# MrGiovanni/R-Super

Hardware: AMD Instinct MI355X
Metric: CT voxels/sec/node (96³ patch, bs=2/GPU) (higher is better)
Workload: dtype bf16; 1 GPU; R-Super 3D UNet(base 32, 26 classes, BasicBlock/IN) full training step (fwd + masked BCE + Dice loss + bwd + clip + AdamW + EMA), 96^3 patches, batch 2/GPU (BASELINE.json configs[1]); global_batch=2, patch=96, parallelism=dp1, sanity_checks_form=device-side flags read one step late (train_ddp.StepGuard)

## Files before the change

include/rsuper_hip.h:

```cpp
#ifndef RSUPER_HIP_H
#define RSUPER_HIP_H
#include <stddef.h>
#include <stdint.h>
#ifdef __cplusplus
extern "C" {
#endif

#define RSUPER_F32 0
#define RSUPER_BF16 1
#define RSUPER_OK 0
#define RSUPER_ERR_ARG 1
#define RSUPER_ERR_LAUNCH 2
#define RSUPER_ERR_UNSUPPORTED 3
#define RSUPER_ERR_NO_DEVICE 4

const char* rsuper_version(void);
int rsuper_device_check(void);


size_t rsuper_conv3_packed_elems(int dtype, int ka, int kb, int n_cols, int bn);

int rsuper_conv3_pack_weights(int dtype, int mode, const float* wa, const float* wb, int ka, int kb, int na, int nb,
                              int bn, void* packed, void* stream);

// ... 76 lines not shown
int rsuper_maxpool2_fwd(int dtype, const void* x, int ldx, void* y, int ldy, float* part, int blocks,
                        int N, int D, int H, int W, int C, void* stream);
int rsuper_maxpool2_bwd(int dtype, const void* x, int ldx, const void* dy, int lddy, void* dx, int lddx,
                        int N, int D, int H, int W, int C, void* stream);
int rsuper_maxpool2_bwd_add(int dtype, const void* x, int ldx, const void* dy, int lddy, const void* add, int lda, void* dx, int lddx,
                            int N, int D, int H, int W, int C, void* stream);

int rsuper_subsample2_fwd(int dtype, const void* x, int ldx, void* y, int ldy, float* part, int blocks,
                          int N, int D, int H, int W, int C, void* stream);
int rsuper_subsample2_bwd(int dtype, const void* dy, int lddy, void* dx, int lddx, int N, int D, int H, int W, int C, void* stream);

int rsuper_upsample_fwd(int dtype, const void* x, int ldx, void* y, int ldy, float* part, int blocks,
                        int N, int ID, int IH, int IW, int OD, int OH, int OW, int C, void* stream);
int rsuper_upsample_bwd(int dtype, const void* dy, int lddy, void* dx, int lddx,
                        int N, int ID, int IH, int IW, int OD, int OH, int OW, int C, void* stream);

int rsuper_stem_fwd(int dtype, const float* x, const float* w, void* y, int ldy, float* part,
                    int N, int D, int H, int W, int C, void* stream);
int rsuper_stem_wgrad(int dtype, const float* x, const void* dy, int lddy, float* dw, int N, int D, int H, int W, int C, void* stream);

int rsuper_head_fwd(int dtype, const void* x, int ldx, const float* w, const float* b, float* logits, int N, int vox, int C, int K, void* stream);
int rsuper_head_bwd_data(int dtype, const float* dlogits, const float* w, void* dx, int lddx, int N, int vox, int C, int K, void* stream);
int rsuper_head_bwd_weight(int dtype, const void* x, int ldx, const float* dlogits, float* dw, float* db, int N, int vox, int C, int K, void* stream);
int rsuper_head_bwd(int dtype, const void* x, int ldx, const float* dlogits, const float* w, void* dx, int lddx, float* dw, float* db,
                    int N, int vox, int C, int K, void* stream);

int rsuper_plane_partials_fwd(const float* x, size_t xstride, const uint8_t* t, const uint8_t* k, const float* w1, const uint8_t* w2,
                              double* sums, int flags, int planes, size_t V, void* stream);
int rsuper_plane_partials_bwd(const float* x, size_t xstride, const uint8_t* t, const uint8_t* k, const float* w1, const uint8_t* w2,
                              const float* g, float* dx, int flags, int planes, size_t V, void* stream);
// ... 174 lines not shown
```

r-super_amd/csrc/api.hip:

```cpp
#include <string.h>
#include <math.h>
#include <stdlib.h>
#include "common.hpp"
#include "kernels.hpp"
#include "misc.hpp"
#include "loss.hpp"
#include "morph.hpp"
#include "optim.hpp"
#include "../../include/rsuper_hip.h"

#define ST(s) ((hipStream_t)(s))

static inline bool dt_ok(int dt) { return dt == RS_F32 || dt == RS_BF16; }
static inline bool ch_ok(int C, int ld) { return C >= 0 && (C % 8) == 0 && (ld % 8) == 0 && ld >= C; }
static inline bool bn_ok(int bn) { return bn == 32 || bn == 64 || bn == 96 || bn == 128; }
static inline int ntiles_for(int n_cols, int bn) { const int per = bn / 32; return ((n_cols + bn - 1) / bn) * per; }
static inline int pack_cols(int mode, int na, int nb) { return mode == 1 ? (nb ? (nb & 0xFFFF) : na) : na + nb; }
static inline bool pack_range_ok(int mode, int na, int nb) { return mode != 1 || nb == 0 || ((nb >> 16) % 32 == 0 && (nb & 0xFFFF) > 0 && (nb >> 16) + (nb & 0xFFFF) <= na); }

#include "igemm_plan.hpp"

template <typename F>
static int for_chunks(int n, void* const* p, void* const* g, void* const* m, void* const* v, void* const* e, const size_t* numel, F f) {
    for (int i0 = 0; i0 < n; i0 += RS_MT_MAX) {
// ... 400 lines not shown
    return rs_launch_subsample(p, dtype, 1, 1, ST(stream));
}

int rsuper_upsample_fwd(int dtype, const void* x, int ldx, void* y, int ldy, float* part, int blocks,
                        int N, int ID, int IH, int IW, int OD, int OH, int OW, int C, void* stream) {
    if (!dt_ok(dtype) || !x || !y || !ch_ok(C, ldx) || !ch_ok(C, ldy) || blocks <= 0) return RS_ERR_ARG;
    UpParams p = {x, ldx, y, ldy, nullptr, 0, part, N, ID, IH, IW, OD, OH, OW, C};
    return rs_launch_upsample(p, dtype, 0, blocks, ST(stream));
}
int rsuper_upsample_bwd(int dtype, const void* dy, int lddy, void* dx, int lddx,
                        int N, int ID, int IH, int IW, int OD, int OH, int OW, int C, void* stream) {
    if (!dt_ok(dtype) || !dy || !dx || !ch_ok(C, lddy) || !ch_ok(C, lddx)) return RS_ERR_ARG;
    UpParams p = {nullptr, 0, (void*)dy, lddy, dx, lddx, nullptr, N, ID, IH, IW, OD, OH, OW, C};
    return rs_launch_upsample(p, dtype, 1, 1, ST(stream));
}
int rsuper_stem_fwd(int dtype, const float* x, const float* w, void* y, int ldy, float* part,
                    int N, int D, int H, int W, int C, void* stream) {
    if (!dt_ok(dtype) || !x || !w || !y || !part || !ch_ok(C, ldy)) return RS_ERR_ARG;
    StemParams p = {x, w, y, ldy, part, nullptr, N, D, H, W, C};
    return rs_launch_stem(p, dtype, 0, ST(stream));
}
int rsuper_stem_wgrad(int dtype, const float* x, const void* dy, int lddy, float* dw, int N, int D, int H, int W, int C, void* stream) {
    if (!dt_ok(dtype) || !x || !dy || !dw || !ch_ok(C, lddy)) return RS_ERR_ARG;
    StemParams p = {x, nullptr, (void*)dy, lddy, nullptr, dw, N, D, H, W, C};
    return rs_launch_stem(p, dtype, 1, ST(stream));
}

int rsuper_head_fwd(int dtype, const void* x, int ldx, const float* w, const float* b, float* logits, int N, int vox, int C, int K, void* stream) {
    if (!dt_ok(dtype) || !x || !w || !b || !logits || !ch_ok(C, ldx) || K <= 0) return RS_ERR_ARG;
    HeadParams p = {x, ldx, w, b, logits, nullptr, 0, nullptr, nullptr, N, vox, C, K};
// ... 342 lines not shown
```

r-super_amd/csrc/misc.hpp:

```cpp
#pragma once
#include <hip/hip_runtime.h>
#include <stddef.h>
#include <stdint.h>

struct InBwdParams {
    const void* g; int ldg;
    const void* x; int ldx;
    const float* mr;
    const float* gm;
    const void* add1; int lda1;
    const void* add2; int lda2;
    void* out; int ldo;
    int N, vox, C;
};

struct PoolParams {
    const void* x; int ldx;
    void* y; int ldy;
    void* dx; int lddx;
    float* part;
    int N, D, H, W, C;
    const void* add; int lda;
};

struct UpParams {
    const void* x; int ldx;
    void* y; int ldy;
    void* dx; int lddx;
    float* part;
    int N, ID, IH, IW, OD, OH, OW, C;
};

struct StemParams {
    const float* x;
    const float* w;
    void* y; int ldy;
    float* part;
    float* dw;
    int N, D, H, W, C;
};

struct HeadParams {
    const void* x; int ldx;
    const float* w; const float* b;
    float* logits;
// ... 15 lines not shown
                         float* hbuf, float* y, int N, long vox, int C, int r, hipStream_t st);
int rs_launch_se_backward(const float* x, const float* dy, const float* ident, const float* w1, const float* w2, const float* ms, const float* tab,
                          const float* hbuf, float* part, float* gm, float* dz1buf, float* tab2, float* dx, float* dw1, float* db1, float* dw2,
                          float* db2, int N, long vox, int C, int r, hipStream_t st);
int rs_launch_cl_planar(const float* src, float* dst, int N, long vox, int C, int K, int dir, hipStream_t st);
int rs_depthwise_rows(long vox);
int rs_launch_depthwise(const float* x, const float* w, float* y, int N, int D, int H, int W, int C, int flip, hipStream_t st);
int rs_launch_depthwise_wgrad(const float* x, const float* dy, float* part, float* dw, int N, int D, int H, int W, int C, hipStream_t st);
int rs_launch_stats_finalize(const float* part, int N, int nblk, int C, double cnt, float eps, int mode, int split, float* out, hipStream_t st);
int rs_elem_blocks(size_t items);
int rs_glue_variant(int v);
int rs_launch_in_bwd(const InBwdParams& p, int dtype, hipStream_t st);
int rs_launch_pool(const PoolParams& p, int dtype, int bwd, int blocks, hipStream_t st);
int rs_launch_subsample(const PoolParams& p, int dtype, int bwd, int blocks, hipStream_t st);
int rs_launch_upsample(const UpParams& p, int dtype, int bwd, int blocks, hipStream_t st);
int rs_launch_stem(const StemParams& p, int dtype, int wgrad, hipStream_t st);
int rs_launch_head(const HeadParams& p, int dtype, int which, hipStream_t st);
```

r-super_amd/csrc/unet_misc.hip:

```cpp
#include <string.h>
#include "common.hpp"
#include "kernels.hpp"
#include "misc.hpp"

namespace {

__global__ __launch_bounds__(1024) void stats_finalize_kernel(const float* part, int nblk, int C, double cnt, float eps, int mode, int split, float* out) {
    __shared__ double red[32][32][2];
    const int n = blockIdx.y;
    const int cl = threadIdx.x & 31, g = threadIdx.x >> 5;
    const int c = blockIdx.x * 32 + cl;
    double s0 = 0.0, s1 = 0.0;
    if (c < C) {
        const float* base = part + ((size_t)n * nblk * C + c) * 2;
        int b = g;
        for (; b + 96 < nblk; b += 128) {
            const float2 v0 = *(const float2*)(base + (size_t)b * C * 2), v1 = *(const float2*)(base + (size_t)(b + 32) * C * 2);
            const float2 v2 = *(const float2*)(base + (size_t)(b + 64) * C * 2), v3 = *(const float2*)(base + (size_t)(b + 96) * C * 2);
            s0 += ((double)v0.x + (double)v1.x) + ((double)v2.x + (double)v3.x);
            s1 += ((double)v0.y + (double)v1.y) + ((double)v2.y + (double)v3.y);
        }
        for (; b < nblk; b += 32) {
            const float2 v = *(const float2*)(base + (size_t)b * C * 2);
            s0 += (double)v.x; s1 += (double)v.y;
// ... 420 lines not shown
    return w;
}

struct UpAxis { int lo, n; float w[6]; };
__device__ __forceinline__ UpAxis up_axis(int i, float scale, int I, int O) {
    UpAxis a;
    int hi;
    up_range(i, scale, O, a.lo, hi);
    a.n = hi - a.lo + 1;
    if (a.n > 6) a.n = 6;
#pragma unroll
    for (int k = 0; k < 6; ++k) a.w[k] = k < a.n ? up_weight(a.lo + k, i, scale, I) : 0.f;
    return a;
}

template <typename T>
__global__ void upsample_bwd_kernel(UpParams p) {
    constexpr int KP = Elem<T>::KP;
    const int CV = p.C / KP;
    const int n = blockIdx.y;
    const size_t total = (size_t)p.ID * p.IH * p.IW * CV;
    const int ovox = p.OD * p.OH * p.OW;
    const float sd = p.OD > 1 ? (float)(p.ID - 1) / (float)(p.OD - 1) : 0.f;
    const float sh = p.OH > 1 ? (float)(p.IH - 1) / (float)(p.OH - 1) : 0.f;
    const float sw = p.OW > 1 ? (float)(p.IW - 1) / (float)(p.OW - 1) : 0.f;
    for (size_t i = (size_t)blockIdx.x * blockDim.x + threadIdx.x; i < total; i += (size_t)gridDim.x * blockDim.x) {
        const int s = (int)(i % CV); const int v = (int)(i / CV);
        const int iw = v % p.IW, ih = (v / p.IW) % p.IH, id = v / (p.IW * p.IH);
        const UpAxis ad = up_axis(id, sd, p.ID, p.OD), ah = up_axis(ih, sh, p.IH, p.OH), aw = up_axis(iw, sw, p.IW, p.OW);
        float acc[KP];
// ... 6 lines not shown
            for (int b = 0; b < 6; ++b) {
                if (ah.w[b] == 0.f) continue;
                const float wdh = ad.w[a] * ah.w[b];
                const size_t rowo = (size_t)n * ovox + ((size_t)(ad.lo + a) * p.OH + (ah.lo + b)) * p.OW;
#pragma unroll
                for (int c = 0; c < 6; ++c) {
                    if (aw.w[c] == 0.f) continue;
                    float g[KP];
                    unpack16<T>(*(const uint4*)((const T*)p.y + (rowo + aw.lo + c) * p.ldy + s * KP), g);
                    const float wt = wdh * aw.w[c];
#pragma unroll
                    for (int j = 0; j < KP; ++j) acc[j] += wt * g[j];
                }
            }
        }
        *(uint4*)((T*)p.dx + ((size_t)n * p.ID * p.IH * p.IW + v) * p.lddx + s * KP) = pack16<T>(acc);
    }
}

template <typename T>
__global__ __launch_bounds__(256) void upsample_fwd2_kernel(UpParams p) {
    constexpr int KP = Elem<T>::KP;
    const int CV = p.C / KP, VL = 256 / CV;
    const int vl = threadIdx.x / CV, s = threadIdx.x % CV;
    const bool active = vl < VL;
    const int n = blockIdx.y;
    const int ovox = p.OD * p.OH * p.OW;
    const int per_blk = (ovox + gridDim.x - 1) / gridDim.x;
    const int v0 = blockIdx.x * per_blk, v1 = min(ovox, v0 + per_blk);
    const float sd = p.OD > 1 ? (float)(p.ID - 1) / (float)(p.OD - 1) : 0.f;
// ... 187 lines not shown
                for (int c = 0; c < NW; ++c) {
                    const uint32_t off = c < nc ? ((rowo + c) * (uint32_t)p.ldy + s * KP) * (uint32_t)sizeof(T) : 0xFFFFFFFFu;
                    const auto r = __builtin_amdgcn_raw_buffer_load_b128(rs, off, 0, 0);
                    q[c] = make_uint4(r[0], r[1], r[2], r[3]);
                }
#pragma unroll
                for (int c = 0; c < NW; ++c) {
                    float g[KP];
                    unpack16<T>(q[c], g);
                    const float wt = wdh * wc[c];
#pragma unroll
                    for (int j = 0; j < KP; ++j) acc[j] = fmaf(wt, g[j], acc[j]);
                }
            }
        }
        *(uint4*)((T*)p.dx + ((size_t)n * p.ID * p.IH * p.IW + v) * p.lddx + s * KP) = pack16<T>(acc);
    }
}

template <typename T>
__global__ __launch_bounds__(256) void upsample_bwd2_kernel(UpParams p) {
    extern __shared__ __attribute__((aligned(16))) char smem[];
    UpEnt* tab = (UpEnt*)smem;
    __shared__ int nwmax;
    if (threadIdx.x == 0) nwmax = 0;
    __syncthreads();
    const float sd = p.OD > 1 ? (float)(p.ID - 1) / (float)(p.OD - 1) : 0.f;
    const float sh = p.OH > 1 ? (float)(p.IH - 1) / (float)(p.OH - 1) : 0.f;
    const float sw = p.OW > 1 ? (float)(p.IW - 1) / (float)(p.OW - 1) : 0.f;
    for (int t = threadIdx.x; t < p.ID + p.IH + p.IW; t += 256) {
// ... 26 lines not shown
    }
    __syncthreads();
    const UpEnt* td = tab; const UpEnt* th = tab + p.ID; const UpEnt* tw = tab + p.ID + p.IH;
    const uint32_t CV = (uint32_t)p.C / Elem<T>::KP;
    const uint32_t total = (uint32_t)(p.ID * p.IH * p.IW) * CV;
    const uint32_t i0 = blockIdx.x * 256u + threadIdx.x, stride = gridDim.x * 256u;
    if (nwmax <= 4) up_bwd_rows<T, 4>(p, td, th, tw, blockIdx.y, i0, total, stride);
    else if (nwmax <= 6) up_bwd_rows<T, 6>(p, td, th, tw, blockIdx.y, i0, total, stride);
    else up_bwd_rows<T, UP_MAXW>(p, td, th, tw, blockIdx.y, i0, total, stride);
}

struct UpInParams {
    const void* g; int ldg;
    void* dx; int lddx;
    int N, ID, IH, IW, OD, OH, OW, C;
};
#ifndef UP4_SL
#define UP4_SL 2
#endif
constexpr int UP4_ROWS = 16;
template <int NT>
__global__ __launch_bounds__(256, 3) void upsample_bwd4_kernel(UpInParams p, int nbx) {
    typedef bf16_t T;
    constexpr int CPT = 8, NWD = CPT / 2;
    constexpr int SL = UP4_SL;
    __shared__ float Wd[UP4_ROWS][2], Wh[UP4_ROWS][2];
    __shared__ float4 W4[UP4_ROWS * UP4_ROWS];
    __shared__ int span[4];
    const int tid = threadIdx.x, n = blockIdx.y;
    const int CV = p.C / CPT, tiles_h = (p.IH + 1) / 2;
// ... 94 lines not shown
            }
            float t[CPT];
#pragma unroll
            for (int j = 0; j < NWD; ++j) { t[2 * j] = tg[j][0]; t[2 * j + 1] = tg[j][1]; }
            const float4 w4 = W4[rr];
            const float wv[4] = {w4.x, w4.y, w4.z, w4.w};
#pragma unroll
            for (int i = 0; i < 4; ++i)
#pragma unroll
                for (int k = 0; k < CPT; ++k) acc[i][k] = fmaf(wv[i], t[k], acc[i][k]);
        }
    }
#pragma unroll
    for (int i = 0; i < 4; ++i) {
        const int id = id0 + (i >> 1), ih = ih0 + (i & 1);
        if (id < p.ID && ih < p.IH)
            *(uint4*)((T*)p.dx + ((size_t)((n * p.ID + id) * p.IH + ih) * p.IW + iw) * p.lddx + s * CPT) = pack16<T>(acc[i]);
    }
}
static int up_max_count(int I, int O) {
    const float sc = O > 1 ? (float)(I - 1) / (float)(O - 1) : 0.f;
    int m = 1;
    for (int i = 0; i < I; ++i) {
        int lo, hi;
        up_range(i, sc, O, lo, hi);
        int first = -1, last = -2;
        for (int o = lo; o <= hi; ++o)
            if (up_weight(o, i, sc, I) != 0.f) { if (first < 0) first = o; last = o; }
        if (last - first + 1 > m) m = last - first + 1;
    }
    return m;
}
static int up_pair_window(int I, int O) {
    const float sc = O > 1 ? (float)(I - 1) / (float)(O - 1) : 0.f;
    int m = 1;
    for (int i = 0; i < I; i += 2) {
        int lo, hi, lo2, hi2;
        up_range(i, sc, O, lo, hi);
        if (i + 1 < I) { up_range(i + 1, sc, O, lo2, hi2); if (hi2 > hi) hi = hi2; }
        if (hi - lo + 1 > m) m = hi - lo + 1;
    }
    return m;
}

template <typename T, int C>
__global__ __launch_bounds__(256) void stem_fwd_kernel(StemParams p) {
    extern __shared__ __attribute__((aligned(16))) char smem[];
    float* tile = (float*)smem;
    const float* __restrict__ w = p.w;
    const int n = blockIdx.y;
    const int vox = p.D * p.H * p.W;
    const int v = blockIdx.x * 256 + threadIdx.x;
    const bool ok = v < vox;
    float xv[27];
    {
        const int x0 = v % p.W, y0 = (v / p.W) % p.H, z0 = v / (p.W * p.H);
        const float* xin = p.x + (size_t)n * vox;
// ... 457 lines not shown
    if (CV > 256) return RS_ERR_UNSUPPORTED;
    if (!bwd) {
        const size_t smem = (size_t)(256 / CV) * p.C * 2 * sizeof(float);
        const int z = stat_csplit(blocks, p.N, CV);
        const dim3 grid(blocks, p.N, z), blk(z == 1 ? 256 : (CV / z) * (256 / CV));
        if (dtype == RS_F32) hipLaunchKernelGGL(subsample_fwd_kernel<float>, grid, blk, smem / z, st, p);
        else hipLaunchKernelGGL(subsample_fwd_kernel<bf16_t>, grid, blk, smem / z, st, p);
    } else {
        const int b = rs_elem_blocks((size_t)p.D * p.H * p.W * CV);
        if (dtype == RS_F32) hipLaunchKernelGGL(subsample_bwd_kernel<float>, dim3(b, p.N), dim3(256), 0, st, p);
        else hipLaunchKernelGGL(subsample_bwd_kernel<bf16_t>, dim3(b, p.N), dim3(256), 0, st, p);
    }
    return rs_check_launch();
}

static int launch_upsample_bwd4(const void* g, int ldg, void* dx, int lddx, int N, int ID, int IH, int IW, int OD, int OH, int OW, int C, hipStream_t st) {
    static const bool off = getenv("RSUPER_UPSAMPLE_BWD4") && atoi(getenv("RSUPER_UPSAMPLE_BWD4")) == 0;
    if (off || (C % 8) || N > 65535) return RS_ERR_UNSUPPORTED;
    if ((size_t)OD * OH * OW * (size_t)ldg * 2 >= 0xFFFFFFFFull) return RS_ERR_UNSUPPORTED;
    struct Memo { int k[6]; int ok, nmax; };
    static thread_local Memo memo[8] = {};
    static thread_local int memo_next = 0;
    const int key[6] = {ID, IH, IW, OD, OH, OW};
    const Memo* hit = nullptr;
    for (int i = 0; i < 8 && !hit; ++i) if (memo[i].k[0] && !memcmp(memo[i].k, key, sizeof(key))) hit = &memo[i];
    if (!hit) {
        Memo& m = memo[memo_next++ & 7];
        memcpy(m.k, key, sizeof(key));
        m.ok = up_pair_window(ID, OD) <= UP4_ROWS && up_pair_window(IH, OH) <= UP4_ROWS;
        m.nmax = up_max_count(IW, OW);
        hit = &m;
    }
    if (!hit->ok) return RS_ERR_UNSUPPORTED;
    const int nmax = hit->nmax;
    if (nmax > 6) return RS_ERR_UNSUPPORTED;
    UpInParams p = {g, ldg, dx, lddx, N, ID, IH, IW, OD, OH, OW, C};
    const int nbx = (IW * (C / 8) + 255) / 256;
    const unsigned blocks = (unsigned)(((ID + 1) / 2) * ((IH + 1) / 2) * nbx);
    if (nmax <= 4) hipLaunchKernelGGL((upsample_bwd4_kernel<4>), dim3(blocks, N), dim3(256), 0, st, p, nbx);
    else hipLaunchKernelGGL((upsample_bwd4_kernel<6>), dim3(blocks, N), dim3(256), 0, st, p, nbx);
    return rs_check_launch();
}

int rs_launch_upsample(const UpParams& p, int dtype, int bwd, int blocks, hipStream_t st) {
    const int KP = dtype == RS_F32 ? 4 : 8;
    const int CV = p.C / KP;
    if (CV > 256) return RS_ERR_UNSUPPORTED;
    if (!bwd) {
        static const bool v1 = getenv("RSUPER_UPSAMPLE_V1") != nullptr;
        const size_t smem = (size_t)(256 / CV) * p.C * 2 * sizeof(float);
        const bool small = (size_t)p.N * p.ID * p.IH * p.IW * p.ldx < 0x7FFFFFFFull;
// ... 8 lines not shown
            if (dtype == RS_F32) hipLaunchKernelGGL(upsample_fwd3_kernel<float>, grid, blk, smem / z + tab3, st, p);
            else hipLaunchKernelGGL(upsample_fwd3_kernel<bf16_t>, grid, blk, smem / z + tab3, st, p);
        } else {
            if (dtype == RS_F32) hipLaunchKernelGGL(upsample_fwd2_kernel<float>, dim3(blocks, p.N), dim3(256), smem, st, p);
            else hipLaunchKernelGGL(upsample_fwd2_kernel<bf16_t>, dim3(blocks, p.N), dim3(256), smem, st, p);
        }
    } else {
        static const bool v1 = getenv("RSUPER_UPSAMPLE_V1") != nullptr;
        auto ratio = [](int O, int I) { return I > 1 ? (double)(O - 1) / (double)(I - 1) : (double)O; };
        const double rmax = fmax(ratio(p.OD, p.ID), fmax(ratio(p.OH, p.IH), ratio(p.OW, p.IW)));
        if (!v1 && 2.0 * rmax + 2.0 > (double)UP_MAXW + 1e-9) return RS_ERR_UNSUPPORTED;
        const int b = rs_elem_blocks((size_t)p.ID * p.IH * p.IW * CV);
        const size_t tab = (size_t)(p.ID + p.IH + p.IW) * sizeof(UpEnt);
        const bool small = (size_t)p.OD * p.OH * p.OW * p.ldy * (dtype == RS_F32 ? 4 : 2) < 0xFFFFFFFFull && (size_t)p.ID * p.IH * p.IW * CV < 0xFFFFFFFFull && tab <= 48 * 1024;
        if (!v1 && dtype == RS_BF16) {
            const int rc = launch_upsample_bwd4(p.y, p.ldy, p.dx, p.lddx, p.N, p.ID, p.IH, p.IW, p.OD, p.OH, p.OW, p.C, st);
            if (rc != RS_ERR_UNSUPPORTED) return rc;
        }
        if (v1 || !small) {
            if (dtype == RS_F32) hipLaunchKernelGGL(upsample_bwd_kernel<float>, dim3(b, p.N), dim3(256), 0, st, p);
            else hipLaunchKernelGGL(upsample_bwd_kernel<bf16_t>, dim3(b, p.N), dim3(256), 0, st, p);
        } else {
            if (dtype == RS_F32) hipLaunchKernelGGL(upsample_bwd2_kernel<float>, dim3(b, p.N), dim3(256), tab, st, p);
            else hipLaunchKernelGGL(upsample_bwd2_kernel<bf16_t>, dim3(b, p.N), dim3(256), tab, st, p);
        }
    }
    return rs_check_launch();
}

#define RS_DISPATCH_C(KERNEL, T, C, ...)                                                        \
    switch (C) {                                                                                \
        case 8: { auto k = KERNEL<T, 8>; set_smem(k, smem); hipLaunchKernelGGL(k, __VA_ARGS__); break; }   \
        case 16: { auto k = KERNEL<T, 16>; set_smem(k, smem); hipLaunchKernelGGL(k, __VA_ARGS__); break; } \
        case 32: { auto k = KERNEL<T, 32>; set_smem(k, smem); hipLaunchKernelGGL(k, __VA_ARGS__); break; } \
        case 64: { auto k = KERNEL<T, 64>; set_smem(k, smem); hipLaunchKernelGGL(k, __VA_ARGS__); break; } \
        default: return RS_ERR_UNSUPPORTED;                                                     \
    }

static float* small_ws(int which) {
    static float* ws[16][2] = {};
    int dev = 0;
    if (hipGetDevice(&dev) != hipSuccess || dev < 0 || dev >= 16) return nullptr;
// ... 69 lines not shown
```

r-super_amd/hip/lib.py:

```python
import ctypes
import os
from ctypes import c_int, c_long, c_longlong, c_size_t, c_float, c_double, c_void_p, c_uint32, c_uint, c_ulonglong

_HERE = os.path.dirname(os.path.abspath(__file__))
SO_PATH = os.path.join(os.path.dirname(_HERE), 'csrc', 'librsuper_hip.so')

F32, BF16 = 0, 1
BLUR_MAX_RADIUS = 5
_LIB = None

P = c_void_p
_SIGS = {
    'rsuper_version': (ctypes.c_char_p, []),
    'rsuper_device_check': (c_int, []),
    'rsuper_conv3_packed_elems': (c_size_t, [c_int] * 5),
    'rsuper_conv3_pack_weights': (c_int, [c_int, c_int, P, P, c_int, c_int, c_int, c_int, c_int, P, P]),
    'rsuper_conv3_pack_weights_batch': (c_int, [c_int, c_int, P, P, P, P, P, P]),
    'rsuper_conv3_tiles': (c_int, [c_int] * 3),
    'rsuper_conv3_variant': (c_int, [c_int]),
    'rsuper_conv3_wgrad2_min_tiles': (c_int, [c_int]),
    'rsuper_conv3_plan': (c_int, [c_int] * 11 + [P]),
    'rsuper_conv3_box_bn': (c_int, [c_int] * 6),
    'rsuper_conv3_kd_bn': (c_int, [c_int] * 8),
    'rsuper_conv3_set_workspace': (c_int, [P, c_size_t]),
# ... 18 lines not shown
    'rsuper_pointwise_packed_bytes': (c_size_t, [c_int, c_int, c_int]),
    'rsuper_pointwise': (c_int, [c_int, c_int, P, c_int, P, P, P, c_int, P, c_int, c_long, c_int, c_int, P, P]),
    'rsuper_pointwise_pack_batch': (c_int, [c_int, P, c_int, c_long, P, P]),
    'rsuper_pointwise_wgrad_splits': (c_int, [c_long, c_int, c_int]),
    'rsuper_pointwise_wgrad': (c_int, [c_int, P, c_int, P, c_int, c_long, c_int, c_int, P, c_int, P, P, P]),
    'rsuper_stats_finalize': (c_int, [P, c_int, c_int, c_int, c_double, c_float, c_int, c_int, P, P]),
    'rsuper_glue_variant': (c_int, [c_int]),
    'rsuper_in_bwd_finalize': (c_int, [c_int, P, c_int, P, c_int, P, P, P, c_int, P, c_int, P, c_int, c_int, c_int, c_int, P]),
    'rsuper_maxpool2_fwd': (c_int, [c_int, P, c_int, P, c_int, P, c_int, c_int, c_int, c_int, c_int, c_int, P]),
    'rsuper_maxpool2_bwd': (c_int, [c_int, P, c_int, P, c_int, P, c_int, c_int, c_int, c_int, c_int, c_int, P]),
    'rsuper_maxpool2_bwd_add': (c_int, [c_int, P, c_int, P, c_int, P, c_int, P, c_int, c_int, c_int, c_int, c_int, c_int, P]),
    'rsuper_subsample2_fwd': (c_int, [c_int, P, c_int, P, c_int, P, c_int, c_int, c_int, c_int, c_int, c_int, P]),
    'rsuper_subsample2_bwd': (c_int, [c_int, P, c_int, P, c_int, c_int, c_int, c_int, c_int, c_int, P]),
    'rsuper_upsample_fwd': (c_int, [c_int, P, c_int, P, c_int, P, c_int] + [c_int] * 8 + [P]),
    'rsuper_upsample_bwd': (c_int, [c_int, P, c_int, P, c_int] + [c_int] * 8 + [P]),
    'rsuper_stem_fwd': (c_int, [c_int, P, P, P, c_int, P, c_int, c_int, c_int, c_int, c_int, P]),
    'rsuper_stem_wgrad': (c_int, [c_int, P, P, c_int, P, c_int, c_int, c_int, c_int, c_int, P]),
    'rsuper_head_fwd': (c_int, [c_int, P, c_int, P, P, P, c_int, c_int, c_int, c_int, P]),
    'rsuper_head_bwd_data': (c_int, [c_int, P, P, P, c_int, c_int, c_int, c_int, c_int, P]),
    'rsuper_head_bwd_weight': (c_int, [c_int, P, c_int, P, P, P, c_int, c_int, c_int, c_int, P]),
    'rsuper_head_bwd': (c_int, [c_int, P, c_int, P, P, P, c_int, P, P, c_int, c_int, c_int, c_int, P]),
    'rsuper_plane_partials_fwd': (c_int, [P, c_size_t, P, P, P, P, P, c_int, c_int, c_size_t, P]),
    'rsuper_plane_partials_fwd2': (c_int, [P, c_size_t, P, P, c_int, c_int, P, P, P, P, P, c_int, c_int, c_size_t, P]),
    'rsuper_plane_partials_fwd3': (c_int, [P, c_size_t, P, P, c_int, c_int, P, P, P, P, P, c_int, c_int, c_size_t, P]),
    'rsuper_plane_partials_blocks': (c_int, [c_size_t]),
    'rsuper_plane_sums_reduce': (c_int, [P, c_int, c_int, P, P]),
    'rsuper_plane_partials_bwd2': (c_int, [P, c_size_t, P, P, c_int, c_int, P, P, P, P, P, P, c_int, c_int, c_size_t, P]),
    'rsuper_cnorm_rows': (c_int, [c_long]),
    'rsuper_cnorm_small': (c_int, [P, P, P, P, P, c_int, c_long, c_int, c_int, c_float, c_int, P]),
    'rsuper_cnorm_forward': (c_int, [P, P, P, P, c_int, c_long, c_int, c_int, c_float, P]),
# ... 124 lines not shown
```

r-super_amd/hip/library.py:

```python
import torch

from . import ops as _ops

LIB = torch.library.Library('rsuper', 'DEF')


class _Ctx:
    needs_input_grad = ()

    def save_for_backward(self, *ts):
        pass

    def mark_non_differentiable(self, *ts):
        pass

    def set_materialize_grads(self, v):
        pass


def _register_plain(name, schema, fn):
    LIB.define(name + schema)
    LIB.impl(name, fn, 'CUDA')
    return getattr(torch.ops.rsuper, name)

# ... 28 lines not shown


def _bb_apply_args(xa, mra, xb, mrb, w1, w2, ws, packs=None, stride=1):
    return xa, mra, xb, mrb, w1, w2, ws, (None if packs is None else list(packs[0])), (None if packs is None else list(packs[1])), stride


def install():
    if getattr(_ops, '_LIBRARY_INSTALLED', False):
        return
    reg = [
        ('BasicBlockFn', 'basic_block',
         '(Tensor xa, Tensor mra, Tensor? xb, Tensor? mrb, Tensor w1, Tensor w2, Tensor? ws, Tensor[]? pack_bufs, int[]? pack_bns, int stride) -> (Tensor, Tensor)',
         _bb_fn_args, _bb_apply_args),
        ('MaxPoolFn', 'maxpool2', '(Tensor x) -> (Tensor, Tensor)', None, None),
        ('MaxPoolSkipFn', 'maxpool2_skip', '(Tensor(a) x) -> (Tensor, Tensor, Tensor(a))', None, None),
        ('UpsampleFn', 'upsample_trilinear', '(Tensor x, int[] size) -> (Tensor, Tensor)', lambda x, size: (x, tuple(size)), None),
        ('StemFn', 'stem_conv', '(Tensor img, Tensor w, ScalarType dtype) -> (Tensor, Tensor)', None, None),
        ('HeadFn', 'head_conv', '(Tensor x, Tensor w, Tensor b) -> Tensor', None, None),
        ('Conv3Fn', 'conv3', '(Tensor x, Tensor w) -> Tensor', None, None),
        ('PlanarFn', 'cl_planar', '(Tensor x, int K) -> Tensor', None, None),
        ('SqueezeExciteFn', 'squeeze_excite', '(Tensor x, Tensor w1, Tensor b1, Tensor w2, Tensor b2) -> Tensor', None, None),
        ('BidirAttnFn', 'bidir_attention', '(Tensor fqv, Tensor mqv, int heads, float scale) -> (Tensor, Tensor)', None, None),
        ('TokenAttnFn', 'token_attention', '(Tensor qkv, int heads, float scale) -> Tensor', None, None),
        ('ChannelNormFn', 'channel_norm', '(Tensor x, float eps, bool relu) -> Tensor', None, None),
        ('DepthwiseConvFn', 'depthwise_conv3', '(Tensor x, Tensor w) -> Tensor', None, None),
    ]
    for cls, name, schema, to_fn, adapt in reg:
        Fn = getattr(_ops, cls)
        op = _register(name, schema, Fn, to_fn)
        setattr(_ops, '_' + cls, Fn)
        setattr(_ops, cls, _Apply(op, adapt, Fn.__doc__))
# ... 153 lines not shown
```

r-super_amd/hip/ops.py:

```python
import ctypes
import os

import torch
import torch.nn.functional as F

from . import lib as _l

EPS = 1e-4
_DT = {torch.float32: _l.F32, torch.bfloat16: _l.BF16}


def use_tr():
    return int(os.environ.get('RSUPER_WGRAD_TR', '1'))


_DEV_INDEX = None


def _stream():
    global _DEV_INDEX
    if _DEV_INDEX is None:
        _DEV_INDEX = torch.cuda.current_device()
    return torch._C._cuda_getCurrentRawStream(_DEV_INDEX)

# ... 538 lines not shown
            ys2 = torch.empty((2, N, D, H, W, Cout), device=dev, dtype=dt)
            ys, sc_t = ys2[0], ys2[1]
            igemm(0, sa, sb, wp1, nc1, bn1, dims, ys, part=part, out2=sc_t, out_split=Cout)
        else:
            ys = torch.empty((N, D, H, W, nc1), device=dev, dtype=dt)
            igemm(0, sa, sb, wp1, nc1, bn1, dims, ys, part=part)
        mr_y1 = stats_finalize(part, cnt, split=Cout)[0] if has_sc else stats_finalize(part, cnt)
        bn2, wp2 = packs[1][1], packs[0][1]
        out = torch.empty((N, D, H, W, Cout), device=dev, dtype=dt)
        part2 = part_buffer(dt, dims, Cout, bn2, dev)
        res = (Src(sc_t) if split_ys else Src(ys, C=Cout, off=Cout)) if has_sc else Src(xa)
        igemm(0, Src(ys, C=Cout, mr=mr_y1), None, wp2, Cout, bn2, dims, out, res=res, part=part2)
        mr_out = stats_finalize(part2, cnt)
        ctx.save_for_backward(xa, mra, xb, mrb, ys, mr_y1, w1, w2, ws)
        ctx.packs = packs if (packs is not None and len(packs[0]) >= 4) else None
        ctx.mark_non_differentiable(mr_out)
        ctx.set_materialize_grads(False)
        return out, mr_out

    @staticmethod
    def _forward_s2(ctx, xa, mra, w1, w2, ws):
        _chk_act(xa)
        assert ws is not None, 'a strided BasicBlock always has a convolutional shortcut (conv_layers.py:82-84)'
        N, D, H, W, Ca = xa.shape
        Cout = w1.shape[0]
        dims = (N, D, H, W)
        dev, dt = xa.device, xa.dtype
        tiles = _L().rsuper_conv3_tiles(D, H, W)
        sa = Src(xa, mr=mra)
        nc1 = 2 * Cout
# ... 11 lines not shown
            wp1 = pack_weights(dt, 0, w1, ws, Ca, 0, Cout, Cout, 64)
            ys = torch.empty((N, OD, OH, OW, nc1), device=dev, dtype=dt)
            part1 = torch.empty((N, _L().rsuper_conv3_s2_part_rows(_DT[dt], 1, Ca, 0, nc1, N, D, H, W), nc1, 2), device=dev, dtype=torch.float32)
            igemm_s2(1, sa, None, wp1, nc1, dims, ys, part1)
            mr_y1 = stats_finalize(part1, OD * OH * OW, split=Cout)[0]
        dims2 = (N, OD, OH, OW)
        tiles2 = _L().rsuper_conv3_tiles(OD, OH, OW)
        bn2 = pick_bn(Cout, dt, tiles2 * N, dims2, epi=0)
        wp2 = pack_weights(dt, 0, w2, None, Cout, 0, Cout, 0, bn2)
        out = torch.empty((N, OD, OH, OW, Cout), device=dev, dtype=dt)
        part2 = part_buffer(dt, dims2, Cout, bn2, dev)
        igemm(0, Src(ys, C=Cout, mr=mr_y1), None, wp2, Cout, bn2, dims2, out, res=Src(ys, C=Cout, off=Cout), part=part2)
        mr_out = stats_finalize(part2, OD * OH * OW)
        ctx.save_for_backward(xa, mra, None, None, ys, mr_y1, w1, w2, ws)
        ctx.packs = None
        ctx.stride = 2
        ctx.mark_non_differentiable(mr_out)
        ctx.set_materialize_grads(False)
        return out, mr_out

    @staticmethod
    def _backward_s2(ctx, dout):
        xa, mra, _, _, ys, mr_y1, w1, w2, ws = ctx.saved_tensors
        dout = dout.contiguous()
        N, D, H, W, Ca = xa.shape
        Cout = w1.shape[0]
        OD, OH, OW = ys.shape[1:4]
        dims, dims2 = (N, D, H, W), (N, OD, OH, OW)
        dev, dt = xa.device, xa.dtype
        y1 = Src(ys, C=Cout, mr=mr_y1)
# ... 101 lines not shown
            igemm(1, Src(dy1), sdo if has_sc else None, wpd1, Cin, bn, dims, g0, part=part0, ea=sa, eb=sb)
            if fuse:
                pending.append((part0, cnt, 1, 0 if xb is None else Ca))
            else:
                gm0 = stats_finalize(part0, cnt, mode=1, split=0 if xb is None else Ca)
        dw1 = grad_dest(w1)
        dws = grad_dest(ws) if has_sc else None
        with _Side(ov, (xa, mra, xb, mrb, dy1, dout, dw1, dws)):
            wgrad(sa, sb, Src(dy1), sdo if has_sc else None, dw1, dws, dims, side_reduce=sr, defer=DEFER_WGRAD_REDUCE and not ov)
        if fuse:
            fin = flush_wgrad_reduces(stats=pending)
            gm0 = fin if len(bpk[0]) == 3 else fin[0]
        if xb is None:
            dxa = in_bwd_finalize(Src(g0), sa, gm0, Ca, add1=None if has_sc else dout)
            dxb = None
        elif split_g0:
            dxa = in_bwd_finalize(Src(g0s[0]), sa, gm0[0], Ca)
            dxb = in_bwd_finalize(Src(g0s[1]), sb, gm0[1], Cb)
        else:
            dxa = in_bwd_finalize(Src(g0, C=Ca), sa, gm0[0], Ca)
            dxb = in_bwd_finalize(Src(g0, C=Cb, off=Ca), sb, gm0[1], Cb)
        flush_wgrad_reduces()
        if (ov or sr) and _join_per_block():
            join_side()
        return dxa, None, dxb, None, dw1, dw2, dws, None, None


_BB = BasicBlockFn


# ... 59 lines not shown
    N, D, H, W, C = x.shape
    OD, OH, OW = (D + 1) // 2, (H + 1) // 2, (W + 1) // 2
    y = torch.empty((N, OD, OH, OW, C), device=x.device, dtype=x.dtype)
    blocks = _stat_blocks(OD * OH * OW)
    part = torch.empty((N, blocks, C, 2), device=x.device, dtype=torch.float32) if with_stats else None
    _l.check(_L().rsuper_subsample2_fwd(_DT[x.dtype], _ptr(x), C, _ptr(y), C, _ptr(part), blocks, N, D, H, W, C, _stream()), 'subsample2_fwd')
    return y, (stats_finalize(part, OD * OH * OW) if with_stats else None)


def subsample2_scatter(dy, out, off, dims):
    N, D, H, W = dims
    C = dy.shape[-1]
    _l.check(_L().rsuper_subsample2_bwd(_DT[dy.dtype], _ptr(dy), C, _ptr(out, off), out.shape[-1], N, D, H, W, C, _stream()), 'subsample2_bwd')


class UpsampleFn(torch.autograd.Function):

    @staticmethod
    def forward(ctx, x, size):
        _chk_act(x)
        N, ID, IH, IW, C = x.shape
        OD, OH, OW = size
        y = torch.empty((N, OD, OH, OW, C), device=x.device, dtype=x.dtype)
        blocks = _stat_blocks(OD * OH * OW)
        part = torch.empty((N, blocks, C, 2), device=x.device, dtype=torch.float32)
        _l.check(_L().rsuper_upsample_fwd(_DT[x.dtype], _ptr(x), C, _ptr(y), C, _ptr(part), blocks, N, ID, IH, IW, OD, OH, OW, C, _stream()),
                  'upsample_fwd')
        mr = stats_finalize(part, OD * OH * OW)
        ctx.in_shape = tuple(x.shape)
        ctx.mark_non_differentiable(mr)
        ctx.set_materialize_grads(False)
        return y, mr

    @staticmethod
    def backward(ctx, dy, _unused):
        dy = dy.contiguous()
        N, ID, IH, IW, C = ctx.in_shape
        OD, OH, OW = dy.shape[1:4]
        dx = torch.empty(ctx.in_shape, device=dy.device, dtype=dy.dtype)
        _l.check(_L().rsuper_upsample_bwd(_DT[dy.dtype], _ptr(dy), C, _ptr(dx), C, N, ID, IH, IW, OD, OH, OW, C, _stream()), 'upsample_bwd')
        return dx, None


class StemFn(torch.autograd.Function):

    @staticmethod
    def forward(ctx, img, w, dtype):
        assert img.dim() == 5 and img.shape[1] == 1, 'hot path supports in_chan == 1 (reference configs use 1)'
        img = img.contiguous().float()
        N, _, D, H, W = img.shape
        C = w.shape[0]
        y = torch.empty((N, D, H, W, C), device=img.device, dtype=dtype)
        blocks = -(-(D * H * W) // 256)
        part = torch.empty((N, blocks, C, 2), device=img.device, dtype=torch.float32)
        _l.check(_L().rsuper_stem_fwd(_DT[dtype], _ptr(img), _ptr(w), _ptr(y), C, _ptr(part), N, D, H, W, C, _stream()), 'stem_fwd')
        mr = stats_finalize(part, D * H * W)
# ... 458 lines not shown
```

r-super_amd/model/dim3/unet_utils.py:

```python
import torch
import torch.nn as nn

from .conv_layers import BasicBlock
from ...hip import ops


class _Pool(nn.Module):

    def forward(self, x, with_skip=False):
        return ops.MaxPoolSkipFn.apply(x) if with_skip else ops.MaxPoolFn.apply(x)


class inconv(nn.Module):
    def __init__(self, in_ch, out_ch, kernel_size=(3, 3, 3), block=BasicBlock, norm='in'):
        super().__init__()
        self.conv1 = nn.Conv3d(in_ch, out_ch, kernel_size=3, padding=1, bias=False)
        self.conv2 = block(out_ch, out_ch, kernel_size=kernel_size, norm=norm)

    def forward(self, img, dtype):
        x, mr = ops.StemFn.apply(img, self.conv1.weight, dtype)
        return self.conv2(x, mr)


class down_block(nn.Module):
# ... 22 lines not shown
            blocks = blocks[1:]
        for blk in blocks:
            x, mr = blk(x, mr)
        return (x, mr, skip) if with_skip else (x, mr)


class up_block(nn.Module):
    def __init__(self, in_ch, out_ch, num_block, block=BasicBlock, kernel_size=(3, 3, 3), up_scale=(2, 2, 2), norm='in'):
        super().__init__()
        layers = [block(in_ch + out_ch, out_ch, kernel_size=kernel_size, norm=norm)]
        for _ in range(num_block - 1):
            layers.append(block(out_ch, out_ch, kernel_size=kernel_size, norm=norm))
        self.conv = nn.Sequential(*layers)

    def forward(self, x1, mr1, x2, mr2):
        up, mru = ops.UpsampleFn.apply(x1, tuple(x2.shape[1:4]))
        x, mr = self.conv[0](x2, mr2, up, mru)
        for blk in list(self.conv)[1:]:
            x, mr = blk(x, mr)
        return x, mr
```

Baseline: 172.4 million voxels/s.

## Fuse instance-norm backward of upsampled input into upsample backward at low resolution

```diff
diff --git a/include/rsuper_hip.h b/include/rsuper_hip.h
--- a/include/rsuper_hip.h
+++ b/include/rsuper_hip.h
@@ -114,6 +114,8 @@
                         int N, int ID, int IH, int IW, int OD, int OH, int OW, int C, void* stream);
 int rsuper_upsample_bwd(int dtype, const void* dy, int lddy, void* dx, int lddx,
                         int N, int ID, int IH, int IW, int OD, int OH, int OW, int C, void* stream);
+int rsuper_upsample_bwd_in(int dtype, const void* g, int ldg, const void* x_low, int ldx, const float* mr, const float* gm, float* corr,
+                           void* dx, int lddx, int N, int ID, int IH, int IW, int OD, int OH, int OW, int C, void* stream);
 
 int rsuper_stem_fwd(int dtype, const float* x, const float* w, void* y, int ldy, float* part,
                     int N, int D, int H, int W, int C, void* stream);
diff --git a/r-super_amd/csrc/api.hip b/r-super_amd/csrc/api.hip
--- a/r-super_amd/csrc/api.hip
+++ b/r-super_amd/csrc/api.hip
@@ -438,6 +438,13 @@
     UpParams p = {nullptr, 0, (void*)dy, lddy, dx, lddx, nullptr, N, ID, IH, IW, OD, OH, OW, C};
     return rs_launch_upsample(p, dtype, 1, 1, ST(stream));
 }
+int rsuper_upsample_bwd_in(int dtype, const void* g, int ldg, const void* x_low, int ldx, const float* mr, const float* gm, float* corr,
+                           void* dx, int lddx, int N, int ID, int IH, int IW, int OD, int OH, int OW, int C, void* stream) {
+    if (!dt_ok(dtype) || !g || !x_low || !mr || !gm || !corr || !dx || !ch_ok(C, ldg) || !ch_ok(C, ldx) || !ch_ok(C, lddx) || C == 0) return RS_ERR_ARG;
+    if (N <= 0 || ID < 1 || IH < 1 || IW < 1 || OD < 1 || OH < 1 || OW < 1) return RS_ERR_ARG;
+    UpParams p = {x_low, ldx, (void*)g, ldg, dx, lddx, nullptr, N, ID, IH, IW, OD, OH, OW, C, nullptr, mr};
+    return rs_launch_upsample_bwd_in(p, gm, corr, dtype, ST(stream));
+}
 int rsuper_stem_fwd(int dtype, const float* x, const float* w, void* y, int ldy, float* part,
                     int N, int D, int H, int W, int C, void* stream) {
     if (!dt_ok(dtype) || !x || !w || !y || !part || !ch_ok(C, ldy)) return RS_ERR_ARG;
diff --git a/r-super_amd/csrc/misc.hpp b/r-super_amd/csrc/misc.hpp
--- a/r-super_amd/csrc/misc.hpp
+++ b/r-super_amd/csrc/misc.hpp
@@ -29,6 +29,8 @@
     void* dx; int lddx;
     float* part;
     int N, ID, IH, IW, OD, OH, OW, C;
+    const float* corr;
+    const float* tail_mr;
 };
 
 struct StemParams {
@@ -74,5 +76,6 @@
 int rs_launch_pool(const PoolParams& p, int dtype, int bwd, int blocks, hipStream_t st);
 int rs_launch_subsample(const PoolParams& p, int dtype, int bwd, int blocks, hipStream_t st);
 int rs_launch_upsample(const UpParams& p, int dtype, int bwd, int blocks, hipStream_t st);
+int rs_launch_upsample_bwd_in(const UpParams& p, const float* gm, float* corr, int dtype, hipStream_t st);
 int rs_launch_stem(const StemParams& p, int dtype, int wgrad, hipStream_t st);
 int rs_launch_head(const HeadParams& p, int dtype, int which, hipStream_t st);
diff --git a/r-super_amd/csrc/unet_misc.hip b/r-super_amd/csrc/unet_misc.hip
--- a/r-super_amd/csrc/unet_misc.hip
+++ b/r-super_amd/csrc/unet_misc.hip
@@ -458,6 +458,18 @@
     return a;
 }
 
+template <int KP>
+__device__ __forceinline__ void up_in_tail(float* acc, const float* corr, const float* mr) {
+    float cv[KP];
+#pragma unroll
+    for (int j = 0; j < KP; j += 4) {
+        const float4 q = *(const float4*)(corr + j);
+        cv[j] = q.x; cv[j + 1] = q.y; cv[j + 2] = q.z; cv[j + 3] = q.w;
+    }
+#pragma unroll
+    for (int j = 0; j < KP; ++j) acc[j] = mr[2 * j + 1] * (acc[j] - cv[j]);
+}
+
 template <typename T>
 __global__ void upsample_bwd_kernel(UpParams p) {
     constexpr int KP = Elem<T>::KP;
@@ -494,6 +506,7 @@
                 }
             }
         }
+        if (p.corr) up_in_tail<KP>(acc, p.corr + ((size_t)n * p.ID * p.IH * p.IW + v) * p.C + s * KP, p.tail_mr + ((size_t)n * p.C + s * KP) * 2);
         *(uint4*)((T*)p.dx + ((size_t)n * p.ID * p.IH * p.IW + v) * p.lddx + s * KP) = pack16<T>(acc);
     }
 }
@@ -711,6 +724,7 @@
                 }
             }
         }
+        if (p.corr) up_in_tail<KP>(acc, p.corr + ((size_t)n * p.ID * p.IH * p.IW + v) * p.C + s * KP, p.tail_mr + ((size_t)n * p.C + s * KP) * 2);
         *(uint4*)((T*)p.dx + ((size_t)n * p.ID * p.IH * p.IW + v) * p.lddx + s * KP) = pack16<T>(acc);
     }
 }
@@ -767,6 +781,7 @@
     const void* g; int ldg;
     void* dx; int lddx;
     int N, ID, IH, IW, OD, OH, OW, C;
+    const float* corr; const float* tail_mr;
 };
 #ifndef UP4_SL
 #define UP4_SL 2
@@ -891,8 +906,11 @@
 #pragma unroll
     for (int i = 0; i < 4; ++i) {
         const int id = id0 + (i >> 1), ih = ih0 + (i & 1);
-        if (id < p.ID && ih < p.IH)
-            *(uint4*)((T*)p.dx + ((size_t)((n * p.ID + id) * p.IH + ih) * p.IW + iw) * p.lddx + s * CPT) = pack16<T>(acc[i]);
+        if (id < p.ID && ih < p.IH) {
+            const size_t v = (size_t)((n * p.ID + id) * p.IH + ih) * p.IW + iw;
+            if (p.corr) up_in_tail<CPT>(acc[i], p.corr + v * p.C + s * CPT, p.tail_mr + ((size_t)n * p.C + s * CPT) * 2);
+            *(uint4*)((T*)p.dx + v * p.lddx + s * CPT) = pack16<T>(acc[i]);
+        }
     }
 }
 static int up_max_count(int I, int O) {
@@ -918,6 +936,107 @@
         if (hi - lo + 1 > m) m = hi - lo + 1;
     }
     return m;
+}
+
+struct UpCorrParams {
+    const void* x; int ldx;
+    const float* mr;
+    const float* gm;
+    float* corr;
+    int N, ID, IH, IW, OD, OH, OW, C;
+};
+template <typename T, int R>
+__global__ __launch_bounds__(256) void upsample_in_corr_kernel(UpCorrParams p) {
+    constexpr int KP = Elem<T>::KP;
+    extern __shared__ __attribute__((aligned(16))) char smem[];
+    float4* tab = (float4*)smem;
+    const float sd = p.OD > 1 ? (float)(p.ID - 1) / (float)(p.OD - 1) : 0.f;
+    const float sh = p.OH > 1 ? (float)(p.IH - 1) / (float)(p.OH - 1) : 0.f;
+    const float sw = p.OW > 1 ? (float)(p.IW - 1) / (float)(p.OW - 1) : 0.f;
+    for (int t = threadIdx.x; t < p.ID + p.IH + p.IW; t += 256) {
+        const int axis = t < p.ID ? 0 : (t < p.ID + p.IH ? 1 : 2);
+        const int i = axis == 0 ? t : (axis == 1 ? t - p.ID : t - p.ID - p.IH);
+        const float sc = axis == 0 ? sd : (axis == 1 ? sh : sw);
+        const int I = axis == 0 ? p.ID : (axis == 1 ? p.IH : p.IW), O = axis == 0 ? p.OD : (axis == 1 ? p.OH : p.OW);
+        int lo, hi;
+        up_range(i, sc, O, lo, hi);
+        float al = 0.f, ad = 0.f, au = 0.f, s = 0.f;
+        for (int o = lo; o <= hi; ++o) {
+            const float w0 = up_weight(o, i, sc, I);
+            if (w0 == 0.f) continue;
+            const float wm = i > 0 ? up_weight(o, i - 1, sc, I) : 0.f, wp = i + 1 < I ? up_weight(o, i + 1, sc, I) : 0.f;
+            al = fmaf(w0, wm, al); ad = fmaf(w0, w0, ad); au = fmaf(w0, wp, au); s += w0;
+        }
+        tab[t] = make_float4(al, ad, au, s);
+    }
+    __syncthreads();
+    const uint32_t CV = (uint32_t)p.C / KP, runs = (uint32_t)(p.IW + R - 1) / R;
+    const uint32_t total = (uint32_t)(p.ID * p.IH) * runs * CV;
+    const uint32_t i = blockIdx.x * 256u + threadIdx.x;
+    if (i >= total) return;
+    const uint32_t n = blockIdx.y;
+    const uint32_t s = i % CV, t1 = i / CV, run = t1 % runs, t2 = t1 / runs;
+    const int ih = (int)(t2 % (uint32_t)p.IH), id = (int)(t2 / (uint32_t)p.IH), iw0 = (int)(run * R);
+    const uint32_t c = s * KP;
+    constexpr int NP = KP / 2;
+    f32x2_t mu[NP], rs[NP], m1[NP], m2[NP];
+#pragma unroll
+    for (int j = 0; j < NP; ++j) {
+        const float4 a = *(const float4*)(p.mr + ((size_t)n * p.C + c + 2 * j) * 2), g = *(const float4*)(p.gm + ((size_t)n * p.C + c + 2 * j) * 2);
+        mu[j] = f32x2_t{a.x, a.z}; rs[j] = f32x2_t{a.y, a.w}; m1[j] = f32x2_t{g.x, g.z}; m2[j] = f32x2_t{g.y, g.w};
+    }
+    const float4 ed = tab[id], eh = tab[p.ID + ih];
+    const float cd[3] = {ed.x, ed.y, ed.z}, ch[3] = {eh.x, eh.y, eh.z};
+    int wi[R + 2];
+#pragma unroll
+    for (int k = 0; k < R + 2; ++k) wi[k] = min(max(iw0 - 1 + k, 0), p.IW - 1);
+    f32x2_t S[R + 2][NP];
+#pragma unroll
+    for (int k = 0; k < R + 2; ++k)
+#pragma unroll
+        for (int j = 0; j < NP; ++j) S[k][j] = f32x2_t{0.f, 0.f};
+    const T* xp = (const T*)p.x + (size_t)n * p.ID * p.IH * p.IW * p.ldx + c;
+#pragma unroll
+    for (int a = 0; a < 3; ++a) {
+        const int d = id + a - 1;
+        if (cd[a] == 0.f || d < 0 || d >= p.ID) continue;
+#pragma unroll
+        for (int b = 0; b < 3; ++b) {
+            const int h = ih + b - 1;
+            if (ch[b] == 0.f || h < 0 || h >= p.IH) continue;
+            const float cdh = cd[a] * ch[b];
+            const f32x2_t c2 = {cdh, cdh};
+            const T* row = xp + (size_t)((d * p.IH + h) * p.IW) * p.ldx;
+            uint4 q[R + 2];
+#pragma unroll
+            for (int k = 0; k < R + 2; ++k) q[k] = *(const uint4*)(row + (size_t)wi[k] * p.ldx);
+#pragma unroll
+            for (int k = 0; k < R + 2; ++k) {
+                float x[KP];
+                unpack16<T>(q[k], x);
+#pragma unroll
+                for (int j = 0; j < NP; ++j) S[k][j] = __builtin_elementwise_fma(c2, f32x2_t{x[2 * j], x[2 * j + 1]} - mu[j], S[k][j]);
+            }
+        }
+    }
+    float* op = p.corr + (((size_t)(n * p.ID + id) * p.IH + ih) * p.IW) * p.C + c;
+#pragma unroll
+    for (int r = 0; r < R; ++r) {
+        if (iw0 + r >= p.IW) break;
+        const float4 e = tab[p.ID + p.IH + iw0 + r];
+        const f32x2_t w0 = {e.x, e.x}, w1 = {e.y, e.y}, w2 = {e.z, e.z};
+        const float sv = (ed.w * eh.w) * e.w;
+        const f32x2_t s2 = {sv, sv};
+        float o[KP];
+#pragma unroll
+        for (int j = 0; j < NP; ++j) {
+            const f32x2_t t = __builtin_elementwise_fma(w2, S[r + 2][j], __builtin_elementwise_fma(w1, S[r + 1][j], w0 * S[r][j])) * rs[j];
+            const f32x2_t v = __builtin_elementwise_fma(m2[j], t, m1[j] * s2);
+            o[2 * j] = v[0]; o[2 * j + 1] = v[1];
+        }
+#pragma unroll
+        for (int j = 0; j < KP; j += 4) *(float4*)(op + (size_t)(iw0 + r) * p.C + j) = make_float4(o[j], o[j + 1], o[j + 2], o[j + 3]);
+    }
 }
 
 template <typename T, int C>
@@ -1405,7 +1524,8 @@
     return rs_check_launch();
 }
 
-static int launch_upsample_bwd4(const void* g, int ldg, void* dx, int lddx, int N, int ID, int IH, int IW, int OD, int OH, int OW, int C, hipStream_t st) {
+static int launch_upsample_bwd4(const void* g, int ldg, void* dx, int lddx, int N, int ID, int IH, int IW, int OD, int OH, int OW, int C,
+                                const float* corr, const float* tail_mr, hipStream_t st) {
     static const bool off = getenv("RSUPER_UPSAMPLE_BWD4") && atoi(getenv("RSUPER_UPSAMPLE_BWD4")) == 0;
     if (off || (C % 8) || N > 65535) return RS_ERR_UNSUPPORTED;
     if ((size_t)OD * OH * OW * (size_t)ldg * 2 >= 0xFFFFFFFFull) return RS_ERR_UNSUPPORTED;
@@ -1425,7 +1545,7 @@
     if (!hit->ok) return RS_ERR_UNSUPPORTED;
     const int nmax = hit->nmax;
     if (nmax > 6) return RS_ERR_UNSUPPORTED;
-    UpInParams p = {g, ldg, dx, lddx, N, ID, IH, IW, OD, OH, OW, C};
+    UpInParams p = {g, ldg, dx, lddx, N, ID, IH, IW, OD, OH, OW, C, corr, tail_mr};
     const int nbx = (IW * (C / 8) + 255) / 256;
     const unsigned blocks = (unsigned)(((ID + 1) / 2) * ((IH + 1) / 2) * nbx);
     if (nmax <= 4) hipLaunchKernelGGL((upsample_bwd4_kernel<4>), dim3(blocks, N), dim3(256), 0, st, p, nbx);
@@ -1464,7 +1584,7 @@
         const size_t tab = (size_t)(p.ID + p.IH + p.IW) * sizeof(UpEnt);
         const bool small = (size_t)p.OD * p.OH * p.OW * p.ldy * (dtype == RS_F32 ? 4 : 2) < 0xFFFFFFFFull && (size_t)p.ID * p.IH * p.IW * CV < 0xFFFFFFFFull && tab <= 48 * 1024;
         if (!v1 && dtype == RS_BF16) {
-            const int rc = launch_upsample_bwd4(p.y, p.ldy, p.dx, p.lddx, p.N, p.ID, p.IH, p.IW, p.OD, p.OH, p.OW, p.C, st);
+            const int rc = launch_upsample_bwd4(p.y, p.ldy, p.dx, p.lddx, p.N, p.ID, p.IH, p.IW, p.OD, p.OH, p.OW, p.C, p.corr, p.tail_mr, st);
             if (rc != RS_ERR_UNSUPPORTED) return rc;
         }
         if (v1 || !small) {
@@ -1476,6 +1596,23 @@
         }
     }
     return rs_check_launch();
+}
+
+int rs_launch_upsample_bwd_in(const UpParams& p, const float* gm, float* corr, int dtype, hipStream_t st) {
+    const int KP = dtype == RS_F32 ? 4 : 8;
+    constexpr int R = 4;
+    const int CV = p.C / KP;
+    const size_t tab = (size_t)(p.ID + p.IH + p.IW) * sizeof(float4);
+    const size_t items = (size_t)p.ID * p.IH * ((p.IW + R - 1) / R) * CV;
+    if (CV < 1 || CV > 256 || p.N > 65535 || tab > 48 * 1024 || items >= 0x7FFFFFFFull || (size_t)p.ID * p.IH * p.IW >= 0x7FFFFFFFull) return RS_ERR_UNSUPPORTED;
+    UpCorrParams c = {p.x, p.ldx, p.tail_mr, gm, corr, p.N, p.ID, p.IH, p.IW, p.OD, p.OH, p.OW, p.C};
+    const dim3 grid((unsigned)((items + 255) / 256), p.N);
+    if (dtype == RS_F32) hipLaunchKernelGGL((upsample_in_corr_kernel<float, R>), grid, dim3(256), tab, st, c);
+    else hipLaunchKernelGGL((upsample_in_corr_kernel<bf16_t, R>), grid, dim3(256), tab, st, c);
+    if (const int rc = rs_check_launch()) return rc;
+    UpParams q = p;
+    q.x = nullptr; q.ldx = 0; q.corr = corr;
+    return rs_launch_upsample(q, dtype, 1, 1, st);
 }
 
 #define RS_DISPATCH_C(KERNEL, T, C, ...)                                                        \
diff --git a/r-super_amd/hip/lib.py b/r-super_amd/hip/lib.py
--- a/r-super_amd/hip/lib.py
+++ b/r-super_amd/hip/lib.py
@@ -56,6 +56,7 @@
     'rsuper_subsample2_bwd': (c_int, [c_int, P, c_int, P, c_int, c_int, c_int, c_int, c_int, c_int, P]),
     'rsuper_upsample_fwd': (c_int, [c_int, P, c_int, P, c_int, P, c_int] + [c_int] * 8 + [P]),
     'rsuper_upsample_bwd': (c_int, [c_int, P, c_int, P, c_int] + [c_int] * 8 + [P]),
+    'rsuper_upsample_bwd_in': (c_int, [c_int, P, c_int, P, c_int, P, P, P, P, c_int] + [c_int] * 8 + [P]),
     'rsuper_stem_fwd': (c_int, [c_int, P, P, P, c_int, P, c_int, c_int, c_int, c_int, c_int, P]),
     'rsuper_stem_wgrad': (c_int, [c_int, P, P, c_int, P, c_int, c_int, c_int, c_int, c_int, P]),
     'rsuper_head_fwd': (c_int, [c_int, P, c_int, P, P, P, c_int, c_int, c_int, c_int, P]),
diff --git a/r-super_amd/hip/library.py b/r-super_amd/hip/library.py
--- a/r-super_amd/hip/library.py
+++ b/r-super_amd/hip/library.py
@@ -66,7 +66,8 @@
          _bb_fn_args, _bb_apply_args),
         ('MaxPoolFn', 'maxpool2', '(Tensor x) -> (Tensor, Tensor)', None, None),
         ('MaxPoolSkipFn', 'maxpool2_skip', '(Tensor(a) x) -> (Tensor, Tensor, Tensor(a))', None, None),
-        ('UpsampleFn', 'upsample_trilinear', '(Tensor x, int[] size) -> (Tensor, Tensor)', lambda x, size: (x, tuple(size)), None),
+        ('UpsampleFn', 'upsample_trilinear', '(Tensor x, int[] size, bool sole_norm_source=False) -> (Tensor, Tensor)',
+         lambda x, size, sole_norm_source=False: (x, tuple(size), sole_norm_source), None),
         ('StemFn', 'stem_conv', '(Tensor img, Tensor w, ScalarType dtype) -> (Tensor, Tensor)', None, None),
         ('HeadFn', 'head_conv', '(Tensor x, Tensor w, Tensor b) -> Tensor', None, None),
         ('Conv3Fn', 'conv3', '(Tensor x, Tensor w) -> Tensor', None, None),
diff --git a/r-super_amd/hip/ops.py b/r-super_amd/hip/ops.py
--- a/r-super_amd/hip/ops.py
+++ b/r-super_amd/hip/ops.py
@@ -576,6 +576,8 @@
         mr_out = stats_finalize(part2, cnt)
         ctx.save_for_backward(xa, mra, xb, mrb, ys, mr_y1, w1, w2, ws)
         ctx.packs = packs if (packs is not None and len(packs[0]) >= 4) else None
+        node = xb.grad_fn if (xb is not None and mrb is not None) else None
+        ctx.up_node = node if getattr(node, 'in_tail', False) else None
         ctx.mark_non_differentiable(mr_out)
         ctx.set_materialize_grads(False)
         return out, mr_out
@@ -617,6 +619,7 @@
         mr_out = stats_finalize(part2, OD * OH * OW)
         ctx.save_for_backward(xa, mra, None, None, ys, mr_y1, w1, w2, ws)
         ctx.packs = None
+        ctx.up_node = None
         ctx.stride = 2
         ctx.mark_non_differentiable(mr_out)
         ctx.set_materialize_grads(False)
@@ -748,6 +751,10 @@
         if xb is None:
             dxa = in_bwd_finalize(Src(g0), sa, gm0, Ca, add1=None if has_sc else dout)
             dxb = None
+        elif ctx.up_node is not None:
+            dxa = in_bwd_finalize(Src(g0s[0]) if split_g0 else Src(g0, C=Ca), sa, gm0[0], Ca)
+            dxb = g0s[1] if split_g0 else g0[..., Ca:]
+            ctx.up_node.tail = (dxb, gm0[1], Cb if split_g0 else Cin)
         elif split_g0:
             dxa = in_bwd_finalize(Src(g0s[0]), sa, gm0[0], Ca)
             dxb = in_bwd_finalize(Src(g0s[1]), sb, gm0[1], Cb)
@@ -837,10 +844,14 @@
     _l.check(_L().rsuper_subsample2_bwd(_DT[dy.dtype], _ptr(dy), C, _ptr(out, off), out.shape[-1], N, D, H, W, C, _stream()), 'subsample2_bwd')
 
 
+def up_in_bwd_enabled():
+    return os.environ.get('RSUPER_UP_IN_BWD', '1') != '0'
+
+
 class UpsampleFn(torch.autograd.Function):
 
     @staticmethod
-    def forward(ctx, x, size):
+    def forward(ctx, x, size, sole_norm_source=False):
         _chk_act(x)
         N, ID, IH, IW, C = x.shape
         OD, OH, OW = size
@@ -851,18 +862,32 @@
                   'upsample_fwd')
         mr = stats_finalize(part, OD * OH * OW)
         ctx.in_shape = tuple(x.shape)
+        ctx.in_tail = bool(sole_norm_source) and up_in_bwd_enabled()
+        ctx.tail = None
+        if ctx.in_tail:
+            ctx.save_for_backward(x, mr)
         ctx.mark_non_differentiable(mr)
         ctx.set_materialize_grads(False)
         return y, mr
 
     @staticmethod
     def backward(ctx, dy, _unused):
-        dy = dy.contiguous()
         N, ID, IH, IW, C = ctx.in_shape
         OD, OH, OW = dy.shape[1:4]
         dx = torch.empty(ctx.in_shape, device=dy.device, dtype=dy.dtype)
+        tail, ctx.tail = ctx.tail, None
+        if tail is not None:
+            g, gm, ldg = tail
+            if dy.data_ptr() != g.data_ptr() or dy.stride() != g.stride():
+                raise RuntimeError('UpsampleFn(sole_norm_source=True): the output has a consumer besides the BasicBlock that reads it')
+            x, mr = ctx.saved_tensors
+            corr = torch.empty((N, ID, IH, IW, C), device=dy.device, dtype=torch.float32)
+            _l.check(_L().rsuper_upsample_bwd_in(_DT[dy.dtype], _ptr(g), ldg, _ptr(x), C, _ptr(mr), _ptr(gm), _ptr(corr), _ptr(dx), C,
+                                                 N, ID, IH, IW, OD, OH, OW, C, _stream()), 'upsample_bwd_in')
+            return dx, None, None
+        dy = dy.contiguous()
         _l.check(_L().rsuper_upsample_bwd(_DT[dy.dtype], _ptr(dy), C, _ptr(dx), C, N, ID, IH, IW, OD, OH, OW, C, _stream()), 'upsample_bwd')
-        return dx, None
+        return dx, None, None
 
 
 class StemFn(torch.autograd.Function):
diff --git a/r-super_amd/model/dim3/unet_utils.py b/r-super_amd/model/dim3/unet_utils.py
--- a/r-super_amd/model/dim3/unet_utils.py
+++ b/r-super_amd/model/dim3/unet_utils.py
@@ -60,7 +60,7 @@
         self.conv = nn.Sequential(*layers)
 
     def forward(self, x1, mr1, x2, mr2):
-        up, mru = ops.UpsampleFn.apply(x1, tuple(x2.shape[1:4]))
+        up, mru = ops.UpsampleFn.apply(x1, tuple(x2.shape[1:4]), True)
         x, mr = self.conv[0](x2, mr2, up, mru)
         for blk in list(self.conv)[1:]:
             x, mr = blk(x, mr)
```

Result: no change. 173.1 million voxels/s (median of 6 runs) (+0.4%).
